# pengfeidip/pytorch-faster-rcnn

Measured on NVIDIA B200. Metric: images/sec of RPN proposal+assign+RoIAlign, R50-FPN 800x1333, higher is better.
Workload: dtype f32

## Files before the change

pytorch-faster-rcnn_b200/csrc/assign.cu:

```cuda
#include <cstdlib>
#include <cstring>

#include "common.cuh"
#include "targets_common.cuh"

namespace b2d {

__device__ __forceinline__ void grid_limits(const b2d_level& lv, float img_h, float img_w, int& in_h, int& in_w) {
    const double r = 1.0 / (double)lv.stride;
    in_h = min(lv.H, (int)((double)img_h * r) + 1);
    in_w = min(lv.W, (int)((double)img_w * r) + 1);
}

__device__ __forceinline__ bool load_box(const AssignArgs& p, const b2d_pyramid& pyr, int b, long long i,
                                         long long n_b, Box& bx, const int* __restrict__ s_lim) {
    if (i >= n_b) return false;
    if (!p.use_pyr) {
        const float* src = p.boxes + (long long)b * 4 * p.box_ld;
        bx.x1 = src[i]; bx.y1 = src[p.box_ld + i]; bx.x2 = src[2 * p.box_ld + i]; bx.y2 = src[3 * p.box_ld + i];
        return true;
    }
    int l = 0;
#pragma unroll
    for (int q = 1; q < kMaxLevels; ++q)
// ... 91 lines not shown
    if (p.use_pyr && threadIdx.x < pyr.num_levels)
        grid_limits(pyr.lv[threadIdx.x], p.img_hw[2 * b], p.img_hw[2 * b + 1], s_lim[2 * threadIdx.x], s_lim[2 * threadIdx.x + 1]);
    __syncthreads();

    Box bx[kBoxesPerThread];
    float ba[kBoxesPerThread], best[kBoxesPerThread], veq[kBoxesPerThread];
    int arg[kBoxesPerThread], eq[kBoxesPerThread];
    bool ok[kBoxesPerThread];
    const long long base = ((long long)blockIdx.x * blockDim.x) * kBoxesPerThread + threadIdx.x;
#pragma unroll
    for (int r = 0; r < kBoxesPerThread; ++r) {
        ok[r] = load_box(p, pyr, b, base + (long long)r * blockDim.x, n_b, bx[r], s_lim);
        ba[r] = ok[r] ? area_plus1(bx[r]) : 0.0f;
        best[r] = 0.0f; veq[r] = 0.0f; arg[r] = 0; eq[r] = -1;
    }
    for (int j0 = 0; j0 < K; j0 += kGtChunk) {
        const int kc = min(kGtChunk, K - j0);
        __syncthreads();
        for (int j = threadIdx.x; j < kc; j += blockDim.x) {
            Box t{g[j0 + j], g[p.gt_ld + j0 + j], g[2 * p.gt_ld + j0 + j], g[3 * p.gt_ld + j0 + j]};
            s_gt[j] = t; s_ga[j] = area_plus1(t);
            s_cm[j] = key2f(colmax[(long long)b * p.gt_ld + j0 + j]);
        }
        __syncthreads();
        for (int j = 0; j < kc; ++j) {
            const Box t = s_gt[j];
            const float ta = s_ga[j], cm = s_cm[j];
            const bool cm_ok = cm >= p.min_pos_iou;
            const bool need_all = (j0 + j) == 0 || (cm_ok && cm == 0.0f) || !(ta > 0.0f);
#pragma unroll
            for (int r = 0; r < kBoxesPerThread; ++r) {
                if (!ok[r]) continue;
                const bool hit = fmaxf(bx[r].x1, t.x1) < fminf(bx[r].x2, t.x2) && fmaxf(bx[r].y1, t.y1) < fminf(bx[r].y2, t.y2);
                if (!(hit || need_all || !(ba[r] > 0.0f))) continue;
                const float v = iou_plus1(bx[r], ba[r], t, ta);
                if ((j0 + j) == 0 || v > best[r]) { best[r] = v; arg[r] = j0 + j; }
                if (eq[r] < 0 && cm_ok && v == cm) { eq[r] = j0 + j; veq[r] = v; }
            }
        }
    }
    int64_t* lab = labels + (long long)b * p.out_ld;
    float* oiou = out_iou + (long long)b * p.out_ld;
    int* plist = pos_list ? pos_list + (long long)b * pos_cap : nullptr;
#pragma unroll
    for (int r = 0; r < kBoxesPerThread; ++r) {
        const long long i = base + (long long)r * blockDim.x;
        int64_t out_l = -1;
        float out_v = 0.0f;
        const bool in_range = i < n_b;
        if (ok[r]) {
            int l = -1;
            if (best[r] < p.neg_iou) l = 0;
            if (best[r] >= p.pos_iou) l = 1;
            int a = arg[r];
            out_v = best[r];
            if (eq[r] >= 0) { l = 1; a = eq[r]; out_v = veq[r]; }
            out_l = (l == 1) ? (int64_t)(a + 1) : (int64_t)l;
        }
        if (in_range) { lab[lead + i] = out_l; oiou[lead + i] = out_v; }
        const bool is_pos = in_range && out_l > 0, is_neg = in_range && out_l == 0;
        const unsigned mp = __ballot_sync(0xffffffffu, is_pos), mn = __ballot_sync(0xffffffffu, is_neg);
        if (lane_id() == 0) {
            if (mp) atomicAdd(&s_cnt[0], __popc(mp));
            if (mn) atomicAdd(&s_cnt[1], __popc(mn));
        }
        if (plist) {
            const int slot = warp_alloc(is_pos, &census[4 * b + 2]);
            if (is_pos && slot < pos_cap) plist[slot] = (int)(lead + i);
        }
    }
    if (p.prepend_gt && blockIdx.x == 0) {
        for (int j = threadIdx.x; j < K; j += blockDim.x) {
            lab[j] = j + 1; oiou[j] = 1.0f;
            if (plist) { const int slot = atomicAdd(&census[4 * b + 2], 1); if (slot < pos_cap) plist[slot] = j; }
        }
        if (threadIdx.x == 0) atomicAdd(&s_cnt[0], K);
    }
    __syncthreads();
    if (threadIdx.x < 2 && s_cnt[threadIdx.x]) atomicAdd(&census[4 * b + threadIdx.x], s_cnt[threadIdx.x]);
}


constexpr int kRowAnchors = 4;

__device__ __forceinline__ bool anchor_valid(const AssignArgs& p, const Box& a, int y, int x, int in_h, int in_w,
                                             float img_h, float img_w) {
    bool ok = (y < in_h) && (x < in_w);
    if (p.border >= 0.0f)
        ok = ok && a.x1 >= -p.border && a.y1 >= -p.border && a.x2 < img_w + p.border && a.y2 < img_h + p.border;
    return ok;
}

constexpr int kRectChunks = 4;

__global__ void __launch_bounds__(256) k_colmax_rect(AssignArgs p, b2d_pyramid pyr, uint32_t* __restrict__ colmax,
                                                     int max_a) {
    __shared__ uint32_t s_red[8];
    const int b = blockIdx.y;
    int w = blockIdx.x;
    const int rc = w % kRectChunks; w /= kRectChunks;
    const int a = w % max_a; w /= max_a;
    const int l = w % pyr.num_levels;
    const int j = w / pyr.num_levels;
    if (j >= p.gt_count[b]) return;
    const b2d_level& lv = pyr.lv[l];
    if (a >= lv.A) return;
    const float* g = p.gt + (long long)b * 4 * p.gt_ld;
    const Box t{g[j], g[p.gt_ld + j], g[2 * p.gt_ld + j], g[3 * p.gt_ld + j]};
    const float ta = area_plus1(t);
    const float img_h = p.img_hw[2 * b], img_w = p.img_hw[2 * b + 1];
    int in_h, in_w;
    grid_limits(lv, img_h, img_w, in_h, in_w);
    const float s = lv.stride;
    const float hw = lv.ws[a] / 2.0f, hh = lv.hs[a] / 2.0f, off = lv.center_lt ? 0.0f : s / 2.0f;
    int x0 = 0, x1 = lv.W - 1, y0 = 0, y1 = lv.H - 1;
    if (ta > 0.0f) {
        x0 = max(0, (int)floorf((t.x1 - hw - off) / s) - 1);
        x1 = min(lv.W - 1, (int)ceilf((t.x2 + hw - off) / s) + 1);
        y0 = max(0, (int)floorf((t.y1 - hh - off) / s) - 1);
        y1 = min(lv.H - 1, (int)ceilf((t.y2 + hh - off) / s) + 1);
    }
    const int rw = x1 - x0 + 1;
    uint32_t m = 0u;
    if (rw > 0) {
        const int tx = threadIdx.x % 64, ty = threadIdx.x / 64;
        for (int y = y0 + rc + ty * kRectChunks; y <= y1; y += 4 * kRectChunks) {
            for (int x = x0 + tx; x <= x1; x += 64) {
                const Box an = anchor_at(lv, a, y, x);
                if (!anchor_valid(p, an, y, x, in_h, in_w, img_h, img_w)) continue;
                m = max(m, f2key(iou_plus1(an, area_plus1(an), t, ta) + 0.0f));
            }
        }
    }
    m = __reduce_max_sync(0xffffffffu, m);
    if (lane_id() == 0) s_red[threadIdx.x >> 5] = m;
    __syncthreads();
    if (threadIdx.x == 0) {
        for (int q = 1; q < 8; ++q) m = max(m, s_red[q]);
        if (m) atomicMax(&colmax[(long long)b * p.gt_ld + j], m);
    }
}

__global__ void __launch_bounds__(256) k_label_rows(AssignArgs p, b2d_pyramid pyr, const uint32_t* __restrict__ colmax,
                                                    int64_t* __restrict__ labels, float* __restrict__ out_iou,
                                                    int* __restrict__ census, int* __restrict__ pos_list, int pos_cap) {
    __shared__ Box s_gt[kGtChunk];
    __shared__ float s_ga[kGtChunk];
    __shared__ float s_cm[kGtChunk];
    __shared__ unsigned char s_all[kGtChunk];
    __shared__ int s_cnt[2];
    const int b = blockIdx.y;
    const int K = p.gt_count[b];
    const float* g = p.gt + (long long)b * 4 * p.gt_ld;
    const float img_h = p.img_hw[2 * b], img_w = p.img_hw[2 * b + 1];
    if (threadIdx.x < 2) s_cnt[threadIdx.x] = 0;
    const long long i0 = ((long long)blockIdx.x * blockDim.x + threadIdx.x) * kRowAnchors;
    Box bx[kRowAnchors];
    float ba[kRowAnchors], best[kRowAnchors], veq[kRowAnchors];
    int arg[kRowAnchors], eq[kRowAnchors];
    bool ok[kRowAnchors], live[kRowAnchors];
    float ylo = INFINITY, yhi = -INFINITY;
    {
        int l = -1, a = 0, y = 0, x = 0, in_h = 0, in_w = 0;
        long long lend = -1;
#pragma unroll
        for (int q = 0; q < kRowAnchors; ++q) {
            const long long i = i0 + q;
            live[q] = i < pyr.total;
            ok[q] = false;
            bx[q] = Box{0.f, 0.f, 0.f, 0.f};
            if (live[q]) {
                if (i >= lend) {
                    l = 0;
                    for (int r = 1; r < pyr.num_levels; ++r) if (i >= pyr.lv[r].offset) l = r;
                    const b2d_level& nv = pyr.lv[l];
                    const int li = (int)(i - nv.offset), hw = nv.H * nv.W;
                    a = li / hw;
                    const int r2 = li - a * hw;
                    y = r2 / nv.W; x = r2 - y * nv.W;
                    lend = nv.offset + (long long)nv.A * hw;
                    grid_limits(nv, img_h, img_w, in_h, in_w);
                }
                const b2d_level& lv = pyr.lv[l];
                bx[q] = anchor_at(lv, a, y, x);
                ok[q] = anchor_valid(p, bx[q], y, x, in_h, in_w, img_h, img_w);
                if (++x == lv.W) { x = 0; if (++y == lv.H) { y = 0; ++a; } }
            }
            ba[q] = ok[q] ? area_plus1(bx[q]) : 0.0f;
            if (ok[q]) { ylo = fminf(ylo, bx[q].y1); yhi = fmaxf(yhi, bx[q].y2); }
            best[q] = 0.0f; veq[q] = 0.0f; arg[q] = 0; eq[q] = -1;
        }
    }
    for (int j0 = 0; j0 < K; j0 += kGtChunk) {
        const int kc = min(kGtChunk, K - j0);
        __syncthreads();
        for (int j = threadIdx.x; j < kc; j += blockDim.x) {
            Box t{g[j0 + j], g[p.gt_ld + j0 + j], g[2 * p.gt_ld + j0 + j], g[3 * p.gt_ld + j0 + j]};
            const float ta = area_plus1(t);
            const uint32_t ck = colmax[(long long)b * p.gt_ld + j0 + j];
            const float cm = ck ? fmaxf(key2f(ck), 0.0f) : 0.0f;
            s_gt[j] = t; s_ga[j] = ta; s_cm[j] = cm;
            s_all[j] = ((j0 + j) == 0 || (cm >= p.min_pos_iou && cm == 0.0f) || !(ta > 0.0f)) ? 1 : 0;
        }
        __syncthreads();
        for (int j = 0; j < kc; ++j) {
            const Box t = s_gt[j];
            const bool all = s_all[j] != 0;
            if (!all && !(fmaxf(ylo, t.y1) < fminf(yhi, t.y2))) continue;
            const float ta = s_ga[j], cm = s_cm[j];
            const bool cm_ok = cm >= p.min_pos_iou;
#pragma unroll
            for (int q = 0; q < kRowAnchors; ++q) {
                if (!ok[q]) continue;
                const bool hit = fmaxf(bx[q].x1, t.x1) < fminf(bx[q].x2, t.x2) && fmaxf(bx[q].y1, t.y1) < fminf(bx[q].y2, t.y2);
                if (!(hit || all || !(ba[q] > 0.0f))) continue;
                const float v = iou_plus1(bx[q], ba[q], t, ta);
                if ((j0 + j) == 0 || v > best[q]) { best[q] = v; arg[q] = j0 + j; }
                if (eq[q] < 0 && cm_ok && v == cm) { eq[q] = j0 + j; veq[q] = v; }
            }
        }
    }
    int64_t* lab = labels + (long long)b * p.out_ld;
    float* oiou = out_iou + (long long)b * p.out_ld;
    int* plist = pos_list ? pos_list + (long long)b * pos_cap : nullptr;
    int64_t ol[kRowAnchors];
    float ov[kRowAnchors];
#pragma unroll
    for (int q = 0; q < kRowAnchors; ++q) {
        ol[q] = -1; ov[q] = 0.0f;
        if (ok[q]) {
            int lb = -1;
            if (best[q] < p.neg_iou) lb = 0;
            if (best[q] >= p.pos_iou) lb = 1;
            int a = arg[q];
            ov[q] = best[q];
            if (eq[q] >= 0) { lb = 1; a = eq[q]; ov[q] = veq[q]; }
            ol[q] = (lb == 1) ? (int64_t)(a + 1) : (int64_t)lb;
        }
    }
    const bool vec = live[kRowAnchors - 1] && ((reinterpret_cast<uintptr_t>(lab) & 15) == 0) &&
                     ((reinterpret_cast<uintptr_t>(oiou) & 15) == 0);
    if (vec) {
        reinterpret_cast<longlong2*>(lab + i0)[0] = make_longlong2(ol[0], ol[1]);
        reinterpret_cast<longlong2*>(lab + i0)[1] = make_longlong2(ol[2], ol[3]);
        *reinterpret_cast<float4*>(oiou + i0) = make_float4(ov[0], ov[1], ov[2], ov[3]);
    } else {
#pragma unroll
        for (int q = 0; q < kRowAnchors; ++q)
            if (live[q]) { lab[i0 + q] = ol[q]; oiou[i0 + q] = ov[q]; }
    }
#pragma unroll
    for (int q = 0; q < kRowAnchors; ++q) {
        const bool is_pos = live[q] && ol[q] > 0, is_neg = live[q] && ol[q] == 0;
        const unsigned mp = __ballot_sync(0xffffffffu, is_pos), mn = __ballot_sync(0xffffffffu, is_neg);
        if (lane_id() == 0) {
            if (mp) atomicAdd(&s_cnt[0], __popc(mp));
            if (mn) atomicAdd(&s_cnt[1], __popc(mn));
        }
        if (plist) {
            const int slot = warp_alloc(is_pos, &census[4 * b + 2]);
            if (is_pos && slot < pos_cap) plist[slot] = (int)(i0 + q);
        }
    }
    __syncthreads();
    if (threadIdx.x < 2 && s_cnt[threadIdx.x]) atomicAdd(&census[4 * b + threadIdx.x], s_cnt[threadIdx.x]);
}

__device__ __forceinline__ void assign_small_body(const AssignArgs& p, SmallSmem& sm, int64_t* __restrict__ labels,
                                                  float* __restrict__ out_iou, int* __restrict__ census,
                                                  int* __restrict__ pos_list, int pos_cap, int* s_lab) {
    Box* s_gt = sm.gt;
    float* s_ga = sm.ga;
    uint32_t* s_max = sm.mx;
    int* s_cnt = sm.cnt;
    const int b = blockIdx.x;
    const int K = p.gt_count[b];
    const int n_b = p.box_count ? p.box_count[b] : (int)p.N;
    const float* g = p.gt + (long long)b * 4 * p.gt_ld;
    const float* src = p.boxes + (long long)b * 4 * p.box_ld;
    const int lead = p.prepend_gt ? K : 0;
    const uint32_t kNegInf = f2key(-INFINITY);
    if (threadIdx.x < 3) s_cnt[threadIdx.x] = 0;
    for (int j = threadIdx.x; j < K; j += blockDim.x) {
        Box t{g[j], g[p.gt_ld + j], g[2 * p.gt_ld + j], g[3 * p.gt_ld + j]};
        s_gt[j] = t; s_ga[j] = area_plus1(t); s_max[j] = kNegInf;
    }
    Box bx[kSmallBoxes];
    float ba[kSmallBoxes];
    bool ok[kSmallBoxes];
#pragma unroll
    for (int r = 0; r < kSmallBoxes; ++r) {
        const int i = threadIdx.x + r * kSmallThreads;
        ok[r] = i < n_b;
        if (ok[r]) bx[r] = Box{src[i], src[p.box_ld + i], src[2 * p.box_ld + i], src[3 * p.box_ld + i]};
        else bx[r] = Box{0.f, 0.f, 0.f, 0.f};
        ba[r] = ok[r] ? area_plus1(bx[r]) : 0.0f;
    }
    __syncthreads();
    for (int j = 0; j < K; ++j) {
        const Box t = s_gt[j];
        const float ta = s_ga[j];
        uint32_t m = kNegInf;
#pragma unroll
        for (int r = 0; r < kSmallBoxes; ++r)
            if (ok[r]) m = max(m, f2key(iou_plus1(bx[r], ba[r], t, ta) + 0.0f));
        m = __reduce_max_sync(0xffffffffu, m);
        if (lane_id() == 0 && m != kNegInf) atomicMax(&s_max[j], m);
    }
    __syncthreads();
    float best[kSmallBoxes], veq[kSmallBoxes];
    int arg[kSmallBoxes], eq[kSmallBoxes];
#pragma unroll
    for (int r = 0; r < kSmallBoxes; ++r) { best[r] = 0.0f; veq[r] = 0.0f; arg[r] = 0; eq[r] = -1; }
    for (int j = 0; j < K; ++j) {
        const Box t = s_gt[j];
        const float ta = s_ga[j], cm = key2f(s_max[j]);
        const bool cm_ok = cm >= p.min_pos_iou;
#pragma unroll
        for (int r = 0; r < kSmallBoxes; ++r) {
            if (!ok[r]) continue;
            const float v = iou_plus1(bx[r], ba[r], t, ta);
            if (j == 0 || v > best[r]) { best[r] = v; arg[r] = j; }
            if (eq[r] < 0 && cm_ok && v == cm) { eq[r] = j; veq[r] = v; }
        }
    }
    int64_t* lab = labels + (long long)b * p.out_ld;
    float* oiou = out_iou + (long long)b * p.out_ld;
    int* plist = pos_list ? pos_list + (long long)b * pos_cap : nullptr;
#pragma unroll
    for (int r = 0; r < kSmallBoxes; ++r) {
        const int i = threadIdx.x + r * kSmallThreads;
        int64_t out_l = -1;
        float out_v = 0.0f;
        if (ok[r]) {
            int l = -1;
            if (best[r] < p.neg_iou) l = 0;
            if (best[r] >= p.pos_iou) l = 1;
            int a = arg[r];
            out_v = best[r];
            if (eq[r] >= 0) { l = 1; a = eq[r]; out_v = veq[r]; }
            out_l = (l == 1) ? (int64_t)(a + 1) : (int64_t)l;
            lab[lead + i] = out_l; oiou[lead + i] = out_v;
            if (s_lab) s_lab[lead + i] = (int)out_l;
        }
        const bool is_pos = ok[r] && out_l > 0, is_neg = ok[r] && out_l == 0;
        const unsigned mp = __ballot_sync(0xffffffffu, is_pos), mn = __ballot_sync(0xffffffffu, is_neg);
        if (lane_id() == 0) {
            if (mp) atomicAdd(&s_cnt[0], __popc(mp));
// ... 262 lines not shown
    if (tar_param) { tar_param[o + t] = prm[0]; tar_param[o + p.max_num + t] = prm[1]; tar_param[o + 2 * p.max_num + t] = prm[2]; tar_param[o + 3 * p.max_num + t] = prm[3]; }
    if (tar_label) tar_label[(long long)b * p.max_num + t] = lab_out;
    if (tar_is_gt) tar_is_gt[(long long)b * p.max_num + t] = isgt;
}

struct GatherArgs {
    const float* cls[kMaxLevels]; const float* reg[kMaxLevels];
    const int* chosen; const int* n_chosen; int max_num, cls_ch;
};

__global__ void __launch_bounds__(128) k_gather_head(GatherArgs p, b2d_pyramid pyr, float* __restrict__ tar_cls,
                                                     float* __restrict__ tar_reg) {
    const int b = blockIdx.y;
    const int t = blockIdx.x * blockDim.x + threadIdx.x;
    if (t >= p.max_num) return;
    const bool live = t < p.n_chosen[b];
    int l = 0, li = 0;
    long long n = 1;
    if (live) {
        const int i = p.chosen[(long long)b * p.max_num + t];
        for (int q = 1; q < pyr.num_levels; ++q) if (i >= pyr.lv[q].offset) l = q;
        li = (int)(i - pyr.lv[l].offset);
        n = (long long)pyr.lv[l].A * pyr.lv[l].H * pyr.lv[l].W;
    }
    for (int c = 0; c < p.cls_ch; ++c)
        tar_cls[((long long)b * p.cls_ch + c) * p.max_num + t] = live ? p.cls[l][((long long)b * p.cls_ch + c) * n + li] : 0.0f;
    for (int c = 0; c < 4; ++c)
        tar_reg[((long long)b * 4 + c) * p.max_num + t] = live ? p.reg[l][((long long)b * 4 + c) * n + li] : 0.0f;
}

__global__ void __launch_bounds__(kSmallThreads) k_roi_targets_small(AssignArgs p, int64_t* __restrict__ labels,
                                                                     float* __restrict__ out_iou,
                                                                     int* __restrict__ census, int* __restrict__ pos_list,
                                                                     int pos_cap, FusedArgs f) {
    __shared__ SmallSmem sm;
    __shared__ FusedScratch fs;
    pdl_wait();
    assign_small_body(p, sm, labels, out_iou, census, pos_list, pos_cap, fs.lab);
    fused_sample_encode(p, f, sm.gt, fs, sm.cnt[0], sm.cnt[1], blockIdx.x);
}

__global__ void k_counter_add(unsigned long long* cell, unsigned long long inc) { *cell += inc; }

__global__ void k_fill_u32(uint32_t* p, uint32_t v, long long n) {
    const long long i = (long long)blockIdx.x * blockDim.x + threadIdx.x;
    if (i < n) p[i] = v;
}

}

using namespace b2d;

extern "C" {

int b2d_assign_max_iou(int64_t* labels, float* max_iou, long long out_ld, const float* boxes, long long box_ld,
                       const int* box_count, long long N, const b2d_pyramid* pyr_host, const float* img_hw,
                       float border, const float* gt, int gt_ld, const int* gt_count, int B, float pos_iou,
                       float neg_iou, float min_pos_iou, int prepend_gt, int* census, int* pos_list, int pos_cap,
                       void* workspace, size_t ws_bytes, void* stream) {
    B2D_REQUIRE(labels && max_iou && gt && gt_count && census, "assign_max_iou: null pointer");
    B2D_REQUIRE(boxes || (pyr_host && img_hw), "assign_max_iou: need boxes or pyramid+img_hw");
    B2D_REQUIRE(B >= 1 && gt_ld >= 1 && N >= 0, "assign_max_iou: bad sizes");
    B2D_REQUIRE(workspace && ws_bytes >= (size_t)B * gt_ld * 4, "assign_max_iou: workspace too small");
    cudaStream_t st = (cudaStream_t)stream;
    AssignArgs a;
    a.boxes = boxes; a.box_ld = box_ld; a.box_count = box_count; a.N = N;
    a.use_pyr = boxes ? 0 : 1; a.img_hw = img_hw; a.border = border;
    a.gt = gt; a.gt_ld = gt_ld; a.gt_count = gt_count;
    a.pos_iou = pos_iou; a.neg_iou = neg_iou; a.min_pos_iou = min_pos_iou;
    a.prepend_gt = prepend_gt; a.out_ld = out_ld;
    b2d_pyramid pyr;
    memset(&pyr, 0, sizeof(pyr));
    if (a.use_pyr) { pyr = *pyr_host; a.N = pyr.total; }
    if (!a.use_pyr && N <= kSmallThreads * kSmallBoxes && gt_ld <= kGtChunk) {
        k_assign_small<<<B, kSmallThreads, 0, st>>>(a, labels, max_iou, census, pos_list, pos_cap);
        return check_launch("assign_max_iou");
    }
    if (a.use_pyr && !prepend_gt && !knobs().assign_old) {
        uint32_t* cmx = (uint32_t*)workspace;
        cudaMemsetAsync(census, 0, sizeof(int) * 4 * B, st);
        cudaMemsetAsync(cmx, 0, sizeof(uint32_t) * (size_t)B * gt_ld, st);
        int max_a = 1;
        for (int l = 0; l < pyr.num_levels; ++l) max_a = max(max_a, pyr.lv[l].A);
        dim3 g1(gt_ld * pyr.num_levels * max_a * kRectChunks, B);
        k_colmax_rect<<<g1, 256, 0, st>>>(a, pyr, cmx, max_a);
        dim3 g2(cdiv(pyr.total, 256 * kRowAnchors), B);
        k_label_rows<<<g2, 256, 0, st>>>(a, pyr, cmx, labels, max_iou, census, pos_list, pos_cap);
        return check_launch("assign_max_iou");
    }
    uint32_t* colmax = (uint32_t*)workspace;
    const long long nc = (long long)B * gt_ld;
    k_fill_u32<<<cdiv(nc, 256), 256, 0, st>>>(colmax, f2key(-INFINITY), nc);
    cudaMemsetAsync(census, 0, sizeof(int) * 4 * B, st);
    const int per_block = 256 * kBoxesPerThread;
    dim3 grid(cdiv(a.N > 0 ? a.N : 1, per_block), B);
    k_assign_colmax<<<grid, 256, 0, st>>>(a, pyr, colmax);
    k_assign_label<<<grid, 256, 0, st>>>(a, pyr, colmax, labels, max_iou, census, pos_list, pos_cap);
    return check_launch("assign_max_iou");
}

int b2d_label_census(int* census, int* pos_list, int pos_cap, const int64_t* labels, long long ld,
                     const int* count, long long n, int B, void* stream) {
    B2D_REQUIRE(census && labels && B >= 1 && n >= 0, "label_census: bad args");
    cudaStream_t st = (cudaStream_t)stream;
    cudaMemsetAsync(census, 0, sizeof(int) * 4 * B, st);
    if (n == 0) return B2D_OK;
    dim3 grid(cdiv(n, 256), B);
    k_label_census<<<grid, 256, 0, st>>>(census, pos_list, pos_cap, labels, ld, count, n);
    return check_launch("label_census");
}

int b2d_sample_labels(int* chosen, int* n_chosen, const int64_t* labels, long long ld, const int* count,
                      const int* count_add, long long n, const int* census, const int* pos_list, int pos_cap, int B, int max_num,
                      int pos_num, unsigned long long seed, const unsigned long long* seed_step, void* stream) {
    B2D_REQUIRE(chosen && n_chosen && labels && census && pos_list, "sample_labels: null pointer");
    B2D_REQUIRE(B >= 1 && max_num >= 1 && max_num <= kSampleSortCap && pos_num >= 0 && pos_num <= max_num,
                "sample_labels: need 1 <= max_num <= 4096 and pos_num <= max_num");
    B2D_REQUIRE(n < (1ll << 31), "sample_labels: n too large");
    B2D_SMEM(k_sample, kSampleSortCap * 8, "k_sample");
    const int threads = (knobs().sample_threads == 128 || knobs().sample_threads == 256) ? knobs().sample_threads : kSampleThreads;
    k_sample<<<B, threads, kSampleSortCap * 8, (cudaStream_t)stream>>>(
        chosen, n_chosen, labels, ld, count, count_add, n, census, pos_list, pos_cap, max_num, pos_num, seed, seed_step);
    return check_launch("sample_labels");
}

int b2d_counter_add(unsigned long long* cell, unsigned long long inc, void* stream) {
    B2D_REQUIRE(cell, "counter_add: null pointer");
    k_counter_add<<<1, 1, 0, (cudaStream_t)stream>>>(cell, inc);
    return check_launch("counter_add");
}

int b2d_scatter_sampled(int64_t* out, const int64_t* labels, long long ld, long long n, const int* chosen,
                        const int* n_chosen, int max_num, int B, void* stream) {
    B2D_REQUIRE(out && labels && chosen && n_chosen && B >= 1, "scatter_sampled: bad args");
    (void)n;
    dim3 grid(cdiv(max_num, 256), B);
    k_scatter_sampled<<<grid, 256, 0, (cudaStream_t)stream>>>(out, labels, ld, chosen, n_chosen, max_num);
    return check_launch("scatter_sampled");
}

int b2d_gather_head_outputs(float* tar_cls, float* tar_reg, const void* const* cls_ptrs_host,
                            const void* const* reg_ptrs_host, const b2d_pyramid* pyr_host, int cls_channels,
                            const int* chosen, const int* n_chosen, int max_num, int B, void* stream) {
    B2D_REQUIRE(tar_cls && tar_reg && cls_ptrs_host && reg_ptrs_host && pyr_host && chosen && n_chosen,
                "gather_head_outputs: null pointer");
    GatherArgs p;
    memset(&p, 0, sizeof(p));
    for (int l = 0; l < pyr_host->num_levels; ++l) { p.cls[l] = (const float*)cls_ptrs_host[l]; p.reg[l] = (const float*)reg_ptrs_host[l]; }
    p.chosen = chosen; p.n_chosen = n_chosen; p.max_num = max_num; p.cls_ch = cls_channels;
    dim3 grid(cdiv(max_num, 128), B);
    k_gather_head<<<grid, 128, 0, (cudaStream_t)stream>>>(p, *pyr_host, tar_cls, tar_reg);
    return check_launch("gather_head_outputs");
}

int b2d_encode_targets(float* tar_box, float* tar_gt, float* tar_param, int64_t* tar_label, int64_t* tar_is_gt,
                       const int* chosen, const int* n_chosen, int max_num, const int64_t* labels,
                       long long label_ld, const float* boxes, long long box_ld, const b2d_pyramid* pyr_host,
                       const float* gt, int gt_ld, const int* gt_count, const int64_t* gt_label, int prepend_gt,
                       const float* means_host, const float* stds_host, int B, void* stream) {
    B2D_REQUIRE(chosen && n_chosen && labels && gt && gt_count, "encode_targets: null pointer");
    B2D_REQUIRE(boxes || pyr_host, "encode_targets: need boxes or pyramid");
    EncArgs p;
    p.chosen = chosen; p.n_chosen = n_chosen; p.max_num = max_num; p.labels = labels; p.label_ld = label_ld;
    p.boxes = boxes; p.box_ld = box_ld; p.use_pyr = boxes ? 0 : 1;
    p.gt = gt; p.gt_ld = gt_ld; p.gt_count = gt_count; p.gt_label = gt_label; p.prepend_gt = prepend_gt;
    for (int i = 0; i < 4; ++i) { p.ms[i] = means_host ? means_host[i] : 0.0f; p.ms[4 + i] = stds_host ? stds_host[i] : 1.0f; }
    b2d_pyramid pyr;
    memset(&pyr, 0, sizeof(pyr));
    if (p.use_pyr) pyr = *pyr_host;
    dim3 grid(cdiv(max_num, 128), B);
// ... 45 lines not shown
```

pytorch-faster-rcnn_b200/fused.py:

```python
import ctypes
import os

import numpy as np
import torch

from . import _C


def _ptrs(tensors):
    arr = (_C.c_void_p * _C.MAX_LEVELS)()
    for i, t in enumerate(tensors):
        arr[i] = t.data_ptr()
    return arr


def pinned_channels_last(t):
    B, C, H, W = t.shape
    h = torch.empty((B, H, W, C), dtype=t.dtype, pin_memory=True).permute(0, 3, 1, 2)
    h.copy_(t)
    return h


def _batch_view(obj, b0, b1, rows_per_image=None):
    import copy
# ... 21 lines not shown
        self.total = int(self.c.total)
        self.level_sizes = [self.num_anchors * g[0] * g[1] for g in self.grids]


class RpnProposals(object):

    def __init__(self, pyramid, B, cfg, means, stds, device, score_mode=0, cls_channels=1, do_nms=True,
                 scale_factor=1.0):
        self.pyr, self.B = pyramid, B
        get = (lambda k, d=0: cfg.get(k, d)) if hasattr(cfg, "get") else (lambda k, d=0: getattr(cfg, k, d))
        c = _C.RpnCfg()
        c.pre_nms, c.post_nms, c.max_num = int(get("pre_nms")), int(get("post_nms")), int(get("max_num"))
        c.score_mode, c.num_cls_channels, c.do_nms = int(score_mode), int(cls_channels), int(bool(do_nms))
        c.nms_thr_f = _C.floor_f32(float(get("nms_iou", 0.7)))
        c.min_size = float(np.float32(scale_factor * get("min_bbox_size", 0)))
        for i in range(4):
            c.means[i], c.stds[i] = float(means[i]), float(stds[i])
        self.cfg = c
        nbytes = _C.lib().b2d_rpn_proposals_workspace_bytes(ctypes.byref(self.pyr.c), B, ctypes.byref(c))
        if nbytes == 0:
            raise _C.B200DetError("rpn_proposals: unsupported configuration (a level needs a pre-NMS top-k <= 16384)")
        self.ws = torch.empty(nbytes, dtype=torch.uint8, device=device)
        post = [(c.post_nms if 0 < c.post_nms < k else k) for k in
                [(c.pre_nms if 0 < c.pre_nms < n else n) for n in pyramid.level_sizes]]
        self.P = c.max_num if c.max_num > 0 else sum(post)
        self.props = torch.zeros((B, 4, self.P), dtype=torch.float32, device=device)
        self.scores = torch.zeros((B, self.P), dtype=torch.float32, device=device)
        self.count = torch.zeros(B, dtype=torch.int32, device=device)
        self.prov = torch.zeros((B, self.P), dtype=torch.int32, device=device)
        self.launches = 0

    def slice(self, b0, b1):
        v = _batch_view(self, b0, b1)
        nbytes = _C.lib().b2d_rpn_proposals_workspace_bytes(ctypes.byref(self.pyr.c), v.B, ctypes.byref(self.cfg))
        v.ws = torch.empty(nbytes, dtype=torch.uint8, device=self.ws.device)
        return v

    def __call__(self, cls_outs, reg_outs, img_hw, records=None, targets=None, after_select=None):
        self.cfg.records = records.data_ptr() if records is not None else None
        self.cfg.event_after_select = after_select.cuda_event if after_select is not None else None
        if targets is not None:
            bt, gt, gt_count, gt_label = targets
            ta = bt.target_args(gt, gt_count, gt_label)
            _C.call("b2d_rpn_proposals_targets", _C.ptr(self.props), _C.ptr(self.scores), _C.ptr(self.count), _C.ptr(self.prov),
                    _ptrs(cls_outs), _ptrs(reg_outs), ctypes.byref(self.pyr.c), _C.ptr(img_hw), self.B,
                    ctypes.byref(self.cfg), _C.ptr(self.ws), self.ws.numel(), ctypes.byref(ta), _C.stream())
            self.launches = int(_C.lib().b2d_last_launch_count())
            return self.props, self.scores, self.count
        _C.call("b2d_rpn_proposals", _C.ptr(self.props), _C.ptr(self.scores), _C.ptr(self.count), _C.ptr(self.prov),
                _ptrs(cls_outs), _ptrs(reg_outs), ctypes.byref(self.pyr.c), _C.ptr(img_hw), self.B,
                ctypes.byref(self.cfg), _C.ptr(self.ws), self.ws.numel(), _C.stream())
        self.launches = int(_C.lib().b2d_last_launch_count())
        return self.props, self.scores, self.count


class BatchedTargets(object):

    def __init__(self, B, n_boxes, gt_ld, assigner, sampler, means, stds, device, pyramid=None, border=0.0,
                 prepend_gt=False, seed=0):
        self.B, self.N, self.gt_ld, self.pyr = B, int(n_boxes), int(gt_ld), pyramid
        self.pos_iou, self.neg_iou, self.min_pos = (np.float32(assigner[k]) for k in ("pos_iou", "neg_iou", "min_pos_iou"))
        self.max_num, self.pos_num = int(sampler["max_num"]), int(sampler["pos_num"])
        self.border, self.prepend, self.seed = float(border), int(bool(prepend_gt)), int(seed)
        self.out_ld = self.N + (self.gt_ld if prepend_gt else 0)
        i32, f32, i64 = torch.int32, torch.float32, torch.int64
        self.labels = torch.empty((B, self.out_ld), dtype=i64, device=device)
        self.iou = torch.empty((B, self.out_ld), dtype=f32, device=device)
        self.census = torch.zeros((B, 4), dtype=i32, device=device)
        self.pos_list = torch.empty((B, self.out_ld), dtype=i32, device=device)
        self.colmax = torch.empty((B, self.gt_ld), dtype=i32, device=device)
        self.chosen = torch.empty((B, self.max_num), dtype=i32, device=device)
        self.n_chosen = torch.zeros(B, dtype=i32, device=device)
        self.tar_box = torch.zeros((B, 4, self.max_num), dtype=f32, device=device)
        self.tar_gt = torch.zeros((B, 4, self.max_num), dtype=f32, device=device)
        self.tar_param = torch.zeros((B, 4, self.max_num), dtype=f32, device=device)
        self.tar_label = torch.zeros((B, self.max_num), dtype=i64, device=device)
        self.tar_is_gt = torch.zeros((B, self.max_num), dtype=i64, device=device)
        self.means, self.stds = _C.host_f4(means, [0, 0, 0, 0]), _C.host_f4(stds, [1, 1, 1, 1])
        self.step_cell = torch.zeros(1, dtype=torch.int64, device=device)
        self.auto_bump = True
        self.b0 = 0
        small = pyramid is None and self.N <= 4096 and self.gt_ld <= 512
        self.fused = small and self.max_num <= 1024
        self.launches = 1 if self.fused else (3 if small else (4 if pyramid is not None else 5))

    def reset_step(self):
        self.step_cell.zero_()

    def target_args(self, gt, gt_count, gt_label):
        assert self.fused
        a = _C.RoiTargetArgs()
        dp = lambda t: t.data_ptr() if t is not None else None
        a.labels, a.max_iou, a.out_ld = dp(self.labels), dp(self.iou), self.out_ld
        a.gt, a.gt_ld, a.gt_count, a.gt_label = dp(gt), self.gt_ld, dp(gt_count), dp(gt_label)
        a.pos_iou, a.neg_iou, a.min_pos_iou = float(self.pos_iou), float(self.neg_iou), float(self.min_pos)
        a.prepend_gt, a.census, a.pos_list, a.pos_cap = self.prepend, dp(self.census), dp(self.pos_list), self.out_ld
        a.chosen, a.n_chosen, a.max_num, a.pos_num = dp(self.chosen), dp(self.n_chosen), self.max_num, self.pos_num
        a.seed = (self.seed * 1000003 + 0x632BE59BD9B4E019 * self.b0) & 0xFFFFFFFFFFFFFFFF
        a.seed_step = dp(self.step_cell)
        a.tar_box, a.tar_gt, a.tar_param = dp(self.tar_box), dp(self.tar_gt), dp(self.tar_param)
        a.tar_label, a.tar_is_gt = dp(self.tar_label), dp(self.tar_is_gt)
        for i in range(4):
            a.means[i], a.stds[i] = self.means[i], self.stds[i]
        return a

    def slice(self, b0, b1):
        return _batch_view(self, b0, b1)

    def __call__(self, gt, gt_count, gt_label=None, boxes=None, box_count=None, img_hw=None, tail_stream=None):
        pyr = ctypes.byref(self.pyr.c) if boxes is None else None
        box_ld = boxes.shape[-1] if boxes is not None else 0
        if self.auto_bump:
            _C.call("b2d_counter_add", _C.ptr(self.step_cell), 1, _C.stream())
        base_seed = (self.seed * 1000003 + 0x632BE59BD9B4E019 * self.b0) & 0xFFFFFFFFFFFFFFFF
        if self.fused and boxes is not None:
            _C.call("b2d_roi_targets_fused", _C.ptr(self.labels), _C.ptr(self.iou), self.out_ld, _C.ptr(boxes), box_ld,
                    _C.ptr(box_count), self.N, _C.ptr(gt), self.gt_ld, _C.ptr(gt_count), _C.ptr(gt_label), self.B,
                    float(self.pos_iou), float(self.neg_iou), float(self.min_pos), self.prepend, _C.ptr(self.census),
                    _C.ptr(self.pos_list), self.out_ld, _C.ptr(self.chosen), _C.ptr(self.n_chosen), self.max_num,
                    self.pos_num, base_seed, _C.ptr(self.step_cell),
                    _C.ptr(self.tar_box), _C.ptr(self.tar_gt), _C.ptr(self.tar_param), _C.ptr(self.tar_label),
                    _C.ptr(self.tar_is_gt), self.means, self.stds, _C.stream())
            return self
        _C.call("b2d_assign_max_iou", _C.ptr(self.labels), _C.ptr(self.iou), self.out_ld, _C.ptr(boxes), box_ld,
                _C.ptr(box_count), self.N, pyr, _C.ptr(img_hw), self.border, _C.ptr(gt), self.gt_ld, _C.ptr(gt_count),
                self.B, float(self.pos_iou), float(self.neg_iou), float(self.min_pos), self.prepend,
                _C.ptr(self.census), _C.ptr(self.pos_list), self.out_ld, _C.ptr(self.colmax), self.colmax.numel() * 4,
                _C.stream())
        cnt, cnt_add = (box_count, gt_count) if (self.prepend and box_count is not None) else \
            ((None, gt_count) if self.prepend else (box_count, None))
        n = self.N if cnt is None else 0
        if tail_stream is not None:
            tail_stream.wait_stream(torch.cuda.current_stream())
            with torch.cuda.stream(tail_stream):
                self._sample_encode(cnt, cnt_add, n, base_seed, boxes, box_ld, pyr, gt, gt_count, gt_label)
            return self
        self._sample_encode(cnt, cnt_add, n, base_seed, boxes, box_ld, pyr, gt, gt_count, gt_label)
        return self

    def _sample_encode(self, cnt, cnt_add, n, base_seed, boxes, box_ld, pyr, gt, gt_count, gt_label):
        _C.call("b2d_sample_labels", _C.ptr(self.chosen), _C.ptr(self.n_chosen), _C.ptr(self.labels), self.out_ld,
                _C.ptr(cnt), _C.ptr(cnt_add), n, _C.ptr(self.census), _C.ptr(self.pos_list), self.out_ld, self.B,
                self.max_num, self.pos_num, base_seed, _C.ptr(self.step_cell), _C.stream())
        _C.call("b2d_encode_targets", _C.ptr(self.tar_box), _C.ptr(self.tar_gt), _C.ptr(self.tar_param),
                _C.ptr(self.tar_label), _C.ptr(self.tar_is_gt), _C.ptr(self.chosen), _C.ptr(self.n_chosen),
                self.max_num, _C.ptr(self.labels), self.out_ld, _C.ptr(boxes), box_ld, pyr, _C.ptr(gt), self.gt_ld,
                _C.ptr(gt_count), _C.ptr(gt_label), self.prepend, self.means, self.stds, self.B, _C.stream())
        return self


class BatchedRoIAlign(object):

    def __init__(self, B, ld, feat_shapes, strides, device, out_size=(7, 7), sampling_ratio=2, finest_scale=56,
                 layout=1):
        cfg = _C.RoiCfg()
        cfg.num_levels, cfg.C = len(strides), int(feat_shapes[0][0])
        cfg.PH, cfg.PW, cfg.sampling_ratio, cfg.aligned = int(out_size[0]), int(out_size[1]), int(sampling_ratio), 0
        cfg.layout, cfg.finest_scale = int(layout), float(finest_scale)
        for l, (s, shp) in enumerate(zip(strides, feat_shapes)):
            cfg.H[l], cfg.W[l], cfg.spatial_scale[l] = int(shp[1]), int(shp[2]), 1.0 / float(s)
        self.cfg, self.B, self.ld = cfg, B, ld
        self.out = torch.zeros((B * ld, cfg.C, cfg.PH, cfg.PW), dtype=torch.float32, device=device)
        self.launches = 1

    def slice(self, b0, b1):
        return _batch_view(self, b0, b1, rows_per_image={"out": self.ld})

# ... 544 lines not shown
```

Measured before the change: 32780.

## Label anchors sparsely via GT rectangles instead of dense all-anchor IoU pass

Replaces the dense row-labelling pass over all pyramid anchors with a sparse scheme. The colmax kernel now also prefills every anchor with the label it gets against the first GT (the default), and a new rect kernel recomputes full labels only for anchors inside each GT's cell rectangle, deduplicating overlapping rectangles. Negative counts are derived analytically from valid row and column counts, and a dense fallback handles degenerate images. Colmax CTAs now loop over GT slices rather than one CTA per GT. This cuts per-anchor all-GT IoU work, at the cost of more complex control flow, an O(j) overlap check per cell, and correctness risk in edge cases.

Result: slower. 27340 (median of 6 runs) (-16.6%).

```diff
diff --git a/pytorch-faster-rcnn_b200/csrc/assign.cu b/pytorch-faster-rcnn_b200/csrc/assign.cu
--- a/pytorch-faster-rcnn_b200/csrc/assign.cu
+++ b/pytorch-faster-rcnn_b200/csrc/assign.cu
@@ -197,6 +197,10 @@
 
 
 constexpr int kRowAnchors = 4;
+constexpr int kRectChunks = 4;
+constexpr int kRectSlices = 8;
+constexpr int kRectGt = 256;
+constexpr int kDenseCtas = 32;
 
 __device__ __forceinline__ bool anchor_valid(const AssignArgs& p, const Box& a, int y, int x, int in_h, int in_w,
                                              float img_h, float img_w) {
@@ -206,105 +210,207 @@
     return ok;
 }
 
-constexpr int kRectChunks = 4;
+__device__ __forceinline__ bool col_valid(const AssignArgs& p, const b2d_level& lv, int a, int x, int in_w, float img_w) {
+    const Box an = anchor_at(lv, a, 0, x);
+    return x < in_w && (p.border < 0.0f || (an.x1 >= -p.border && an.x2 < img_w + p.border));
+}
+__device__ __forceinline__ bool row_valid(const AssignArgs& p, const b2d_level& lv, int a, int y, int in_h, float img_h) {
+    const Box an = anchor_at(lv, a, y, 0);
+    return y < in_h && (p.border < 0.0f || (an.y1 >= -p.border && an.y2 < img_h + p.border));
+}
+
+__device__ __forceinline__ int64_t final_label(const AssignArgs& p, float best, int arg, int eq, float veq, float& out_v) {
+    int lb = -1;
+    if (best < p.neg_iou) lb = 0;
+    if (best >= p.pos_iou) lb = 1;
+    out_v = best;
+    if (eq >= 0) { lb = 1; arg = eq; out_v = veq; }
+    return (lb == 1) ? (int64_t)(arg + 1) : (int64_t)lb;
+}
+
+__device__ __forceinline__ float colmax_of(const uint32_t* __restrict__ colmax, const AssignArgs& p, int b, int j) {
+    const uint32_t ck = colmax[(long long)b * p.gt_ld + j];
+    return ck ? fmaxf(key2f(ck), 0.0f) : 0.0f;
+}
+
+__device__ bool dense_image(const AssignArgs& p, const b2d_pyramid& pyr, const uint32_t* __restrict__ colmax, int b) {
+    const int K = p.gt_count[b];
+    const float* g = p.gt + (long long)b * 4 * p.gt_ld;
+    bool f = K > kRectGt || !(p.pos_iou > 0.0f);
+    for (int j = threadIdx.x; j < K && !f; j += blockDim.x) {
+        const Box t{g[j], g[p.gt_ld + j], g[2 * p.gt_ld + j], g[3 * p.gt_ld + j]};
+        const float ta = area_plus1(t), cm = colmax_of(colmax, p, b, j);
+        f = !(ta > 0.0f) || (cm >= p.min_pos_iou && cm == 0.0f);
+    }
+    for (int l = 0; l < pyr.num_levels; ++l)
+        if (threadIdx.x < pyr.lv[l].A) f = f || !(pyr.lv[l].ws[threadIdx.x] >= 0.0f && pyr.lv[l].hs[threadIdx.x] >= 0.0f);
+    return __syncthreads_or(f) != 0;
+}
+
+struct CellRect { int x0, x1, y0, y1; };
+__device__ __forceinline__ CellRect cell_rect(const b2d_level& lv, int a, const Box& t, float ta) {
+    CellRect r{0, lv.W - 1, 0, lv.H - 1};
+    if (ta > 0.0f) {
+        const float s = lv.stride;
+        const float hw = lv.ws[a] / 2.0f, hh = lv.hs[a] / 2.0f, off = lv.center_lt ? 0.0f : s / 2.0f;
+        const float cw = (float)lv.W + 2.0f, ch = (float)lv.H + 2.0f;
+        r.x0 = max(0, (int)floorf(fminf(fmaxf((t.x1 - hw - off) / s, -2.0f), cw)) - 1);
+        r.x1 = min(lv.W - 1, (int)ceilf(fminf(fmaxf((t.x2 + hw - off) / s, -2.0f), cw)) + 1);
+        r.y0 = max(0, (int)floorf(fminf(fmaxf((t.y1 - hh - off) / s, -2.0f), ch)) - 1);
+        r.y1 = min(lv.H - 1, (int)ceilf(fminf(fmaxf((t.y2 + hh - off) / s, -2.0f), ch)) + 1);
+    }
+    return r;
+}
+
+struct RectCta { int js, l, a, rc; };
+__device__ __forceinline__ RectCta rect_cta(const b2d_pyramid& pyr, int max_a) {
+    int w = blockIdx.x;
+    RectCta c;
+    c.rc = w % kRectChunks; w /= kRectChunks;
+    c.a = w % max_a; w /= max_a;
+    c.l = w % pyr.num_levels;
+    c.js = w / pyr.num_levels;
+    return c;
+}
+
+__device__ __forceinline__ void load_row_group(const AssignArgs& p, const b2d_pyramid& pyr, long long i0,
+                                               float img_h, float img_w, Box (&bx)[kRowAnchors],
+                                               bool (&ok)[kRowAnchors], bool (&live)[kRowAnchors]) {
+    int l = -1, a = 0, y = 0, x = 0, in_h = 0, in_w = 0;
+    long long lend = -1;
+#pragma unroll
+    for (int q = 0; q < kRowAnchors; ++q) {
+        const long long i = i0 + q;
+        live[q] = i < pyr.total;
+        ok[q] = false;
+        bx[q] = Box{0.f, 0.f, 0.f, 0.f};
+        if (live[q]) {
+            if (i >= lend) {
+                l = 0;
+                for (int r = 1; r < pyr.num_levels; ++r) if (i >= pyr.lv[r].offset) l = r;
+                const b2d_level& nv = pyr.lv[l];
+                const int li = (int)(i - nv.offset), hw = nv.H * nv.W;
+                a = li / hw;
+                const int r2 = li - a * hw;
+                y = r2 / nv.W; x = r2 - y * nv.W;
+                lend = nv.offset + (long long)nv.A * hw;
+                grid_limits(nv, img_h, img_w, in_h, in_w);
+            }
+            const b2d_level& lv = pyr.lv[l];
+            bx[q] = anchor_at(lv, a, y, x);
+            ok[q] = anchor_valid(p, bx[q], y, x, in_h, in_w, img_h, img_w);
+            if (++x == lv.W) { x = 0; if (++y == lv.H) { y = 0; ++a; } }
+        }
+    }
+}
+
+__device__ __forceinline__ void store_row_group(int64_t* lab, float* oiou, long long i0, const int64_t (&ol)[kRowAnchors],
+                                                const float (&ov)[kRowAnchors], const bool (&live)[kRowAnchors]) {
+    const bool vec = live[kRowAnchors - 1] && ((reinterpret_cast<uintptr_t>(lab) & 15) == 0) &&
+                     ((reinterpret_cast<uintptr_t>(oiou) & 15) == 0);
+    if (vec) {
+        reinterpret_cast<longlong2*>(lab + i0)[0] = make_longlong2(ol[0], ol[1]);
+        reinterpret_cast<longlong2*>(lab + i0)[1] = make_longlong2(ol[2], ol[3]);
+        *reinterpret_cast<float4*>(oiou + i0) = make_float4(ov[0], ov[1], ov[2], ov[3]);
+    } else {
+#pragma unroll
+        for (int q = 0; q < kRowAnchors; ++q)
+            if (live[q]) { lab[i0 + q] = ol[q]; oiou[i0 + q] = ov[q]; }
+    }
+}
+
+__device__ __forceinline__ void label_fill_block(const AssignArgs& p, const b2d_pyramid& pyr, int64_t* __restrict__ labels,
+                                                 float* __restrict__ out_iou, int b, long long blk) {
+    const int K = p.gt_count[b];
+    const float img_h = p.img_hw[2 * b], img_w = p.img_hw[2 * b + 1];
+    const long long i0 = (blk * blockDim.x + threadIdx.x) * kRowAnchors;
+    Box bx[kRowAnchors];
+    bool ok[kRowAnchors], live[kRowAnchors];
+    load_row_group(p, pyr, i0, img_h, img_w, bx, ok, live);
+    Box t{0.f, 0.f, 0.f, 0.f};
+    float ta = 0.0f;
+    if (K > 0) {
+        const float* g = p.gt + (long long)b * 4 * p.gt_ld;
+        t = Box{g[0], g[p.gt_ld], g[2 * p.gt_ld], g[3 * p.gt_ld]};
+        ta = area_plus1(t);
+    }
+    int64_t ol[kRowAnchors];
+    float ov[kRowAnchors];
+#pragma unroll
+    for (int q = 0; q < kRowAnchors; ++q) {
+        ol[q] = -1; ov[q] = 0.0f;
+        if (ok[q]) {
+            const float v = K > 0 ? iou_plus1(bx[q], area_plus1(bx[q]), t, ta) : 0.0f;
+            ol[q] = final_label(p, v, 0, -1, 0.0f, ov[q]);
+        }
+    }
+    store_row_group(labels + (long long)b * p.out_ld, out_iou + (long long)b * p.out_ld, i0, ol, ov, live);
+}
 
 __global__ void __launch_bounds__(256) k_colmax_rect(AssignArgs p, b2d_pyramid pyr, uint32_t* __restrict__ colmax,
-                                                     int max_a) {
+                                                     int max_a, int rect_ctas, int64_t* __restrict__ labels,
+                                                     float* __restrict__ out_iou) {
     __shared__ uint32_t s_red[8];
     const int b = blockIdx.y;
-    int w = blockIdx.x;
-    const int rc = w % kRectChunks; w /= kRectChunks;
-    const int a = w % max_a; w /= max_a;
-    const int l = w % pyr.num_levels;
-    const int j = w / pyr.num_levels;
-    if (j >= p.gt_count[b]) return;
-    const b2d_level& lv = pyr.lv[l];
-    if (a >= lv.A) return;
+    if ((int)blockIdx.x >= rect_ctas) { label_fill_block(p, pyr, labels, out_iou, b, blockIdx.x - rect_ctas); return; }
+    const RectCta c = rect_cta(pyr, max_a);
+    const int K = p.gt_count[b];
+    const b2d_level& lv = pyr.lv[c.l];
+    if (c.js >= K || c.a >= lv.A) return;
     const float* g = p.gt + (long long)b * 4 * p.gt_ld;
-    const Box t{g[j], g[p.gt_ld + j], g[2 * p.gt_ld + j], g[3 * p.gt_ld + j]};
-    const float ta = area_plus1(t);
     const float img_h = p.img_hw[2 * b], img_w = p.img_hw[2 * b + 1];
     int in_h, in_w;
     grid_limits(lv, img_h, img_w, in_h, in_w);
-    const float s = lv.stride;
-    const float hw = lv.ws[a] / 2.0f, hh = lv.hs[a] / 2.0f, off = lv.center_lt ? 0.0f : s / 2.0f;
-    int x0 = 0, x1 = lv.W - 1, y0 = 0, y1 = lv.H - 1;
-    if (ta > 0.0f) {
-        x0 = max(0, (int)floorf((t.x1 - hw - off) / s) - 1);
-        x1 = min(lv.W - 1, (int)ceilf((t.x2 + hw - off) / s) + 1);
-        y0 = max(0, (int)floorf((t.y1 - hh - off) / s) - 1);
-        y1 = min(lv.H - 1, (int)ceilf((t.y2 + hh - off) / s) + 1);
-    }
-    const int rw = x1 - x0 + 1;
-    uint32_t m = 0u;
-    if (rw > 0) {
-        const int tx = threadIdx.x % 64, ty = threadIdx.x / 64;
-        for (int y = y0 + rc + ty * kRectChunks; y <= y1; y += 4 * kRectChunks) {
-            for (int x = x0 + tx; x <= x1; x += 64) {
-                const Box an = anchor_at(lv, a, y, x);
+    const int tx = threadIdx.x % 64, ty = threadIdx.x / 64;
+    for (int j = c.js; j < K; j += kRectSlices) {
+        const Box t{g[j], g[p.gt_ld + j], g[2 * p.gt_ld + j], g[3 * p.gt_ld + j]};
+        const float ta = area_plus1(t);
+        const CellRect r = cell_rect(lv, c.a, t, ta);
+        uint32_t m = 0u;
+        for (int y = r.y0 + c.rc + ty * kRectChunks; y <= r.y1; y += 4 * kRectChunks) {
+            for (int x = r.x0 + tx; x <= r.x1; x += 64) {
+                const Box an = anchor_at(lv, c.a, y, x);
                 if (!anchor_valid(p, an, y, x, in_h, in_w, img_h, img_w)) continue;
                 m = max(m, f2key(iou_plus1(an, area_plus1(an), t, ta) + 0.0f));
             }
         }
-    }
-    m = __reduce_max_sync(0xffffffffu, m);
-    if (lane_id() == 0) s_red[threadIdx.x >> 5] = m;
-    __syncthreads();
-    if (threadIdx.x == 0) {
-        for (int q = 1; q < 8; ++q) m = max(m, s_red[q]);
-        if (m) atomicMax(&colmax[(long long)b * p.gt_ld + j], m);
-    }
-}
-
-__global__ void __launch_bounds__(256) k_label_rows(AssignArgs p, b2d_pyramid pyr, const uint32_t* __restrict__ colmax,
-                                                    int64_t* __restrict__ labels, float* __restrict__ out_iou,
-                                                    int* __restrict__ census, int* __restrict__ pos_list, int pos_cap) {
+        m = __reduce_max_sync(0xffffffffu, m);
+        if (lane_id() == 0) s_red[threadIdx.x >> 5] = m;
+        __syncthreads();
+        if (threadIdx.x == 0) {
+            for (int q = 1; q < 8; ++q) m = max(m, s_red[q]);
+            if (m) atomicMax(&colmax[(long long)b * p.gt_ld + j], m);
+        }
+        __syncthreads();
+    }
+}
+
+__device__ __forceinline__ void label_rows_block(const AssignArgs& p, const b2d_pyramid& pyr, const uint32_t* __restrict__ colmax,
+                                                 int64_t* __restrict__ labels, float* __restrict__ out_iou,
+                                                 int* __restrict__ census, int* __restrict__ pos_list, int pos_cap,
+                                                 int b, long long blk) {
     __shared__ Box s_gt[kGtChunk];
     __shared__ float s_ga[kGtChunk];
     __shared__ float s_cm[kGtChunk];
     __shared__ unsigned char s_all[kGtChunk];
     __shared__ int s_cnt[2];
-    const int b = blockIdx.y;
+    if (threadIdx.x < 2) s_cnt[threadIdx.x] = 0;
+    __syncthreads();
     const int K = p.gt_count[b];
     const float* g = p.gt + (long long)b * 4 * p.gt_ld;
     const float img_h = p.img_hw[2 * b], img_w = p.img_hw[2 * b + 1];
-    if (threadIdx.x < 2) s_cnt[threadIdx.x] = 0;
-    const long long i0 = ((long long)blockIdx.x * blockDim.x + threadIdx.x) * kRowAnchors;
+    const long long i0 = (blk * blockDim.x + threadIdx.x) * kRowAnchors;
     Box bx[kRowAnchors];
     float ba[kRowAnchors], best[kRowAnchors], veq[kRowAnchors];
     int arg[kRowAnchors], eq[kRowAnchors];
     bool ok[kRowAnchors], live[kRowAnchors];
     float ylo = INFINITY, yhi = -INFINITY;
-    {
-        int l = -1, a = 0, y = 0, x = 0, in_h = 0, in_w = 0;
-        long long lend = -1;
-#pragma unroll
-        for (int q = 0; q < kRowAnchors; ++q) {
-            const long long i = i0 + q;
-            live[q] = i < pyr.total;
-            ok[q] = false;
-            bx[q] = Box{0.f, 0.f, 0.f, 0.f};
-            if (live[q]) {
-                if (i >= lend) {
-                    l = 0;
-                    for (int r = 1; r < pyr.num_levels; ++r) if (i >= pyr.lv[r].offset) l = r;
-                    const b2d_level& nv = pyr.lv[l];
-                    const int li = (int)(i - nv.offset), hw = nv.H * nv.W;
-                    a = li / hw;
-                    const int r2 = li - a * hw;
-                    y = r2 / nv.W; x = r2 - y * nv.W;
-                    lend = nv.offset + (long long)nv.A * hw;
-                    grid_limits(nv, img_h, img_w, in_h, in_w);
-                }
-                const b2d_level& lv = pyr.lv[l];
-                bx[q] = anchor_at(lv, a, y, x);
-                ok[q] = anchor_valid(p, bx[q], y, x, in_h, in_w, img_h, img_w);
-                if (++x == lv.W) { x = 0; if (++y == lv.H) { y = 0; ++a; } }
-            }
-            ba[q] = ok[q] ? area_plus1(bx[q]) : 0.0f;
-            if (ok[q]) { ylo = fminf(ylo, bx[q].y1); yhi = fmaxf(yhi, bx[q].y2); }
-            best[q] = 0.0f; veq[q] = 0.0f; arg[q] = 0; eq[q] = -1;
-        }
+    load_row_group(p, pyr, i0, img_h, img_w, bx, ok, live);
+#pragma unroll
+    for (int q = 0; q < kRowAnchors; ++q) {
+        ba[q] = ok[q] ? area_plus1(bx[q]) : 0.0f;
+        if (ok[q]) { ylo = fminf(ylo, bx[q].y1); yhi = fmaxf(yhi, bx[q].y2); }
+        best[q] = 0.0f; veq[q] = 0.0f; arg[q] = 0; eq[q] = -1;
     }
     for (int j0 = 0; j0 < K; j0 += kGtChunk) {
         const int kc = min(kGtChunk, K - j0);
@@ -312,8 +418,7 @@
         for (int j = threadIdx.x; j < kc; j += blockDim.x) {
             Box t{g[j0 + j], g[p.gt_ld + j0 + j], g[2 * p.gt_ld + j0 + j], g[3 * p.gt_ld + j0 + j]};
             const float ta = area_plus1(t);
-            const uint32_t ck = colmax[(long long)b * p.gt_ld + j0 + j];
-            const float cm = ck ? fmaxf(key2f(ck), 0.0f) : 0.0f;
+            const float cm = colmax_of(colmax, p, b, j0 + j);
             s_gt[j] = t; s_ga[j] = ta; s_cm[j] = cm;
             s_all[j] = ((j0 + j) == 0 || (cm >= p.min_pos_iou && cm == 0.0f) || !(ta > 0.0f)) ? 1 : 0;
         }
@@ -343,27 +448,9 @@
 #pragma unroll
     for (int q = 0; q < kRowAnchors; ++q) {
         ol[q] = -1; ov[q] = 0.0f;
-        if (ok[q]) {
-            int lb = -1;
-            if (best[q] < p.neg_iou) lb = 0;
-            if (best[q] >= p.pos_iou) lb = 1;
-            int a = arg[q];
-            ov[q] = best[q];
-            if (eq[q] >= 0) { lb = 1; a = eq[q]; ov[q] = veq[q]; }
-            ol[q] = (lb == 1) ? (int64_t)(a + 1) : (int64_t)lb;
-        }
-    }
-    const bool vec = live[kRowAnchors - 1] && ((reinterpret_cast<uintptr_t>(lab) & 15) == 0) &&
-                     ((reinterpret_cast<uintptr_t>(oiou) & 15) == 0);
-    if (vec) {
-        reinterpret_cast<longlong2*>(lab + i0)[0] = make_longlong2(ol[0], ol[1]);
-        reinterpret_cast<longlong2*>(lab + i0)[1] = make_longlong2(ol[2], ol[3]);
-        *reinterpret_cast<float4*>(oiou + i0) = make_float4(ov[0], ov[1], ov[2], ov[3]);
-    } else {
-#pragma unroll
-        for (int q = 0; q < kRowAnchors; ++q)
-            if (live[q]) { lab[i0 + q] = ol[q]; oiou[i0 + q] = ov[q]; }
-    }
+        if (ok[q]) ol[q] = final_label(p, best[q], arg[q], eq[q], veq[q], ov[q]);
+    }
+    store_row_group(lab, oiou, i0, ol, ov, live);
 #pragma unroll
     for (int q = 0; q < kRowAnchors; ++q) {
         const bool is_pos = live[q] && ol[q] > 0, is_neg = live[q] && ol[q] == 0;
@@ -379,6 +466,111 @@
     }
     __syncthreads();
     if (threadIdx.x < 2 && s_cnt[threadIdx.x]) atomicAdd(&census[4 * b + threadIdx.x], s_cnt[threadIdx.x]);
+    __syncthreads();
+}
+
+__global__ void __maxnreg__(80) k_label_rect(AssignArgs p, b2d_pyramid pyr, const uint32_t* __restrict__ colmax,
+                                                    int max_a, int64_t* __restrict__ labels, float* __restrict__ out_iou,
+                                                    int* __restrict__ census, int* __restrict__ pos_list, int pos_cap) {
+    __shared__ Box s_gt[kRectGt];
+    __shared__ float s_ga[kRectGt], s_cm[kRectGt];
+    __shared__ CellRect s_rect[kRectGt];
+    const int b = blockIdx.y;
+    const int rect_ctas = gridDim.x - 1 - kDenseCtas;
+    if (dense_image(p, pyr, colmax, b)) {
+        if ((int)blockIdx.x <= rect_ctas) return;
+        const long long nblk = (pyr.total + 256 * kRowAnchors - 1) / (256 * kRowAnchors);
+        for (long long blk = blockIdx.x - rect_ctas - 1; blk < nblk; blk += kDenseCtas)
+            label_rows_block(p, pyr, colmax, labels, out_iou, census, pos_list, pos_cap, b, blk);
+        return;
+    }
+    if ((int)blockIdx.x > rect_ctas) return;
+    const int K = p.gt_count[b];
+    const float img_h = p.img_hw[2 * b], img_w = p.img_hw[2 * b + 1];
+    float miss_v;
+    const int64_t miss = final_label(p, 0.0f, 0, -1, 0.0f, miss_v);
+    if ((int)blockIdx.x == rect_ctas) {
+        if (miss != 0) return;
+        long long valid = 0;
+        for (int l = 0; l < pyr.num_levels; ++l) {
+            const b2d_level& lv = pyr.lv[l];
+            int in_h, in_w;
+            grid_limits(lv, img_h, img_w, in_h, in_w);
+            for (int a = 0; a < lv.A; ++a) {
+                int rows = 0, cols = 0;
+                for (int y = 0; y < lv.H; y += blockDim.x)
+                    rows += __syncthreads_count(y + (int)threadIdx.x < lv.H && row_valid(p, lv, a, y + threadIdx.x, in_h, img_h));
+                for (int x = 0; x < lv.W; x += blockDim.x)
+                    cols += __syncthreads_count(x + (int)threadIdx.x < lv.W && col_valid(p, lv, a, x + threadIdx.x, in_w, img_w));
+                valid += (long long)rows * cols;
+            }
+        }
+        if (threadIdx.x == 0 && valid) atomicAdd(&census[4 * b + 1], (int)valid);
+        return;
+    }
+    const RectCta c = rect_cta(pyr, max_a);
+    const b2d_level& lv = pyr.lv[c.l];
+    if (c.js >= K || c.a >= lv.A) return;
+    const float* g = p.gt + (long long)b * 4 * p.gt_ld;
+    for (int j = threadIdx.x; j < K; j += blockDim.x) {
+        const Box t{g[j], g[p.gt_ld + j], g[2 * p.gt_ld + j], g[3 * p.gt_ld + j]};
+        s_gt[j] = t; s_ga[j] = area_plus1(t); s_cm[j] = colmax_of(colmax, p, b, j);
+        s_rect[j] = cell_rect(lv, c.a, t, s_ga[j]);
+    }
+    __syncthreads();
+    int in_h, in_w;
+    grid_limits(lv, img_h, img_w, in_h, in_w);
+    int64_t* lab = labels + (long long)b * p.out_ld;
+    float* oiou = out_iou + (long long)b * p.out_ld;
+    int* plist = pos_list ? pos_list + (long long)b * pos_cap : nullptr;
+    int n_pos = 0, d_neg = 0;
+    const int tx = threadIdx.x % 64, ty = threadIdx.x / 64;
+    for (int j = c.js; j < K; j += kRectSlices) {
+        const CellRect r = s_rect[j];
+        for (int y = r.y0 + c.rc + ty * kRectChunks; y <= r.y1; y += 4 * kRectChunks) {
+            for (int xb = r.x0; xb <= r.x1; xb += 64) {
+                const int x = xb + tx;
+                const Box an = anchor_at(lv, c.a, y, x);
+                bool mine = x <= r.x1 && anchor_valid(p, an, y, x, in_h, in_w, img_h, img_w);
+                for (int q = 0; q < j && mine; ++q) {
+                    const CellRect o = s_rect[q];
+                    mine = !(x >= o.x0 && x <= o.x1 && y >= o.y0 && y <= o.y1);
+                }
+                int64_t ol = 0;
+                if (mine) {
+                    const float ba = area_plus1(an);
+                    float best = 0.0f, veq = 0.0f;
+                    int arg = 0, eq = -1;
+                    for (int q = 0; q < K; ++q) {
+                        const Box t = s_gt[q];
+                        const bool hit = fmaxf(an.x1, t.x1) < fminf(an.x2, t.x2) && fmaxf(an.y1, t.y1) < fminf(an.y2, t.y2);
+                        if (!(hit || q == 0 || !(ba > 0.0f))) continue;
+                        const float v = iou_plus1(an, ba, t, s_ga[q]), cm = s_cm[q];
+                        if (q == 0 || v > best) { best = v; arg = q; }
+                        if (eq < 0 && cm >= p.min_pos_iou && v == cm) { eq = q; veq = v; }
+                    }
+                    float ov;
+                    ol = final_label(p, best, arg, eq, veq, ov);
+                    const long long i = lv.offset + ((long long)c.a * lv.H + y) * lv.W + x;
+                    lab[i] = ol; oiou[i] = ov;
+                    if (ol > 0) ++n_pos;
+                    d_neg += (ol == 0) - (miss == 0);
+                }
+                if (plist) {
+                    const bool is_pos = mine && ol > 0;
+                    const int slot = warp_alloc(is_pos, &census[4 * b + 2]);
+                    if (is_pos && slot < pos_cap)
+                        plist[slot] = (int)(lv.offset + ((long long)c.a * lv.H + y) * lv.W + x);
+                }
+            }
+        }
+    }
+    n_pos = __reduce_add_sync(0xffffffffu, n_pos);
+    d_neg = __reduce_add_sync(0xffffffffu, d_neg);
+    if (lane_id() == 0) {
+        if (n_pos) atomicAdd(&census[4 * b + 0], n_pos);
+        if (d_neg) atomicAdd(&census[4 * b + 1], d_neg);
+    }
 }
 
 __device__ __forceinline__ void assign_small_body(const AssignArgs& p, SmallSmem& sm, int64_t* __restrict__ labels,
@@ -807,10 +999,11 @@
         cudaMemsetAsync(cmx, 0, sizeof(uint32_t) * (size_t)B * gt_ld, st);
         int max_a = 1;
         for (int l = 0; l < pyr.num_levels; ++l) max_a = max(max_a, pyr.lv[l].A);
-        dim3 g1(gt_ld * pyr.num_levels * max_a * kRectChunks, B);
-        k_colmax_rect<<<g1, 256, 0, st>>>(a, pyr, cmx, max_a);
-        dim3 g2(cdiv(pyr.total, 256 * kRowAnchors), B);
-        k_label_rows<<<g2, 256, 0, st>>>(a, pyr, cmx, labels, max_iou, census, pos_list, pos_cap);
+        const int rect_ctas = min(gt_ld, kRectSlices) * pyr.num_levels * max_a * kRectChunks;
+        const int fill_ctas = cdiv(pyr.total, 256 * kRowAnchors);
+        k_colmax_rect<<<dim3(rect_ctas + fill_ctas, B), 256, 0, st>>>(a, pyr, cmx, max_a, rect_ctas, labels, max_iou);
+        k_label_rect<<<dim3(rect_ctas + 1 + kDenseCtas, B), 256, 0, st>>>(a, pyr, cmx, max_a, labels, max_iou, census,
+                                                                         pos_list, pos_cap);
         return check_launch("assign_max_iou");
     }
     uint32_t* colmax = (uint32_t*)workspace;
diff --git a/pytorch-faster-rcnn_b200/fused.py b/pytorch-faster-rcnn_b200/fused.py
--- a/pytorch-faster-rcnn_b200/fused.py
+++ b/pytorch-faster-rcnn_b200/fused.py
@@ -127,7 +127,7 @@
         self.b0 = 0
         small = pyramid is None and self.N <= 4096 and self.gt_ld <= 512
         self.fused = small and self.max_num <= 1024
-        self.launches = 1 if self.fused else (3 if small else (4 if pyramid is not None else 5))
+        self.launches = 1 if self.fused else (3 if small else (6 if pyramid is not None else 5))
 
     def reset_step(self):
         self.step_cell.zero_()
```
